# cestpasphoto/alpha-zero-general

Hardware: AMD Instinct MI355X
Metric: self-play env-steps/sec @ numMCTSSims=800, Splendor-2p (higher is better)
Workload: dtype f64

## Files before the change

alpha-zero-general_amd/_lib.py:

```python
import ctypes as C
import os

HERE = os.path.dirname(os.path.abspath(__file__))
LIB_PATH = os.environ.get('AZG_LIB') or os.path.join(HERE, 'libazg_hip.so')

SPLENDOR, SANTORINI, AZUL, MINIVILLES, ABALONE, TLP, BOTANIK, AKROPOLIS, SMALLWORLD = 0, 1, 2, 3, 4, 5, 6, 7, 8


class ForestCfg(C.Structure):
    _fields_ = [('game', C.c_int), ('variant', C.c_int), ('n_trees', C.c_int), ('node_capacity', C.c_int),
                ('row_capacity_bytes', C.c_int), ('numMCTSSims', C.c_int), ('cpuct', C.c_double), ('fpu', C.c_double),
                ('universes', C.c_int), ('prob_fullMCTS', C.c_double), ('ratio_fullMCTS', C.c_int),
                ('forced_playouts', C.c_int), ('dirichletAlpha', C.c_double), ('temperature', C.c_double * 3),
                ('tempThreshold', C.c_double), ('rng_seed', C.c_uint64), ('stream0', C.c_uint64),
                ('max_examples', C.c_int), ('level_budget', C.c_int), ('work_budget', C.c_int), ('gc_high_water_pct', C.c_int)]


class SelfplayStats(C.Structure):
    _fields_ = [(n, C.c_uint64) for n in ('plies', 'games', 'sims', 'levels', 'expansions', 'sum_valid_visited',
                                          'terminal_hits', 'examples', 'gc_runs', 'max_nodes', 'errors',
                                          'sum_depth_at_expand', 'cyc_select', 'cyc_levels', 'cyc_edge', 'cyc_leaf')] + [
                                          ('cyc_seg', C.c_uint64 * 4), ('max_live_after_gc', C.c_uint64), ('examples_dropped', C.c_uint64)]


class AzgError(RuntimeError):
    pass


_lib = None

EXPORTS = [
    'azg_last_error', 'azg_version', 'azg_device_count', 'azg_set_device', 'azg_game_info', 'azg_env_valid_moves',
    'azg_env_next_state', 'azg_env_game_ended', 'azg_env_canonical', 'azg_env_init_boards', 'azg_env_symmetries', 'azg_env_symmetries_ex', 'azg_debug_poison_onchip', 'azg_stream_create_xcd', 'azg_stream_destroy', 'azg_debug_placement', 'azg_eval_hashnet', 'azg_forest_create',
    'azg_forest_destroy', 'azg_forest_device_bytes', 'azg_forest_reset', 'azg_forest_begin_search',
    'azg_forest_select', 'azg_forest_select_fused', 'azg_forest_rounds_v80_h2', 'azg_forest_rounds_profile', 'azg_forest_expand_backup', 'azg_forest_active', 'azg_forest_action_probs',
    'azg_forest_root_stats', 'azg_forest_dump_tree', 'azg_forest_validate', 'azg_selfplay_start', 'azg_selfplay_start_ex', 'azg_selfplay_advance', 'azg_selfplay_active',
    'azg_selfplay_stats_get', 'azg_selfplay_drain_examples', 'azg_forest_last_kernel_ms', 'azg_forest_enable_timing', 'azg_forest_set_search_params', 'azg_nn_v80_forward', 'azg_nn_v80_forward_split', 'azg_nn_v80_forward_h2',
    'azg_nn_mb1d_forward', 'azg_nn_mb1d_forward_h2', 'azg_nn_conv5_forward', 'azg_nn_conv5_forward_split', 'azg_nn_conv5_forward_h2', 'azg_nn_s78_forward', 'azg_nn_s78_forward_split', 'azg_nn_s78_forward_h2',
    'azg_nn_aba21_forward', 'azg_nn_sw62_forward', 'azg_nn_akr31_forward', 'azg_nn_bot_forward', 'azg_forest_async_rounds_sw62', 'azg_pick_actions', 'azg_env_playouts',
    'azg_eval_losses', 'azg_train_sample_ids', 'azg_train_gather', 'azg_train_losses',
    'azg_train_adamw', 'azg_train_step_advance', 'azg_examples_expand', 'azg_train_gather_forms',
]


def lib():
    global _lib
    if _lib is not None:
        return _lib
    if not os.path.exists(LIB_PATH):
        raise AzgError('HIP extension %s is missing: run `python __graft_entry__.py build` (hipcc, gfx950). '
                       'There is no CPU fallback.' % LIB_PATH)
    L = C.CDLL(LIB_PATH)
    vp, i, u64, dbl = C.c_void_p, C.c_int, C.c_uint64, C.c_double
    ip = C.POINTER(C.c_int)
    L.azg_last_error.restype = C.c_char_p
    L.azg_version.restype = C.c_char_p
    if hasattr(L, 'azg_forest_cfg_size') and L.azg_forest_cfg_size() != C.sizeof(ForestCfg):
        raise AzgError('%s (%s) has a %d-byte azg_forest_cfg, this binding a %d-byte one: rebuild the library'
                       % (LIB_PATH, L.azg_version().decode(), L.azg_forest_cfg_size(), C.sizeof(ForestCfg)))
    L.azg_game_info.argtypes = [i, i, ip, ip, ip, ip, ip]
    L.azg_env_valid_moves.argtypes = [i, i, vp, vp, i, vp, vp]
    L.azg_env_next_state.argtypes = [i, i, vp, vp, vp, vp, i, vp, vp, u64, u64, vp, vp]
    L.azg_env_game_ended.argtypes = [i, i, vp, vp, i, vp, vp, vp, vp]
    L.azg_env_canonical.argtypes = [i, i, vp, vp, i, vp, vp]
# ... 97 lines not shown
```

alpha-zero-general_amd/csrc/azg_async.hip.h:

```cpp
#pragma once
#include "azg_fused.hip.h"
#include "selfplay.hip.h"

namespace azg {

constexpr uint32_t ERR_ASYNC_TIMEOUT = 128;
constexpr int ASYNC_RING_LAPS = 8;
#ifndef AZG_ASYNC_SEL_WAVES
#define AZG_ASYNC_SEL_WAVES 16
#endif
constexpr int ASYNC_SEL_WAVES = AZG_ASYNC_SEL_WAVES;
#ifndef AZG_ASYNC_SCOUTS
#define AZG_ASYNC_SCOUTS 1
#endif
constexpr uint32_t ASYNC_IDLE_STEP_CAP = 100000u;
#ifndef AZG_IDLE_SLEEP
#define AZG_IDLE_SLEEP 16
#endif
#ifndef AZG_SCOUT_SLEEP
#define AZG_SCOUT_SLEEP 8
#endif
#ifndef AZG_V80_NET_SHARE_256
#define AZG_V80_NET_SHARE_256 136
#endif
// ... 644 lines not shown
                astore(A->ts_ready + (size_t)gi * ASYNC_RS + ii, wall32());
                astore(A->ready + (size_t)gi * ASYNC_RS + ii, (uint32_t)sidx[16 + tid] + 1u);
            }
        }
        if (tid == 0) {
            P[0] += 1ull; P[1] += (unsigned long long)sidx[32]; P[2] += (unsigned long long)(wall32() - (uint32_t)sidx[33]);
            P[5] += (unsigned long long)((uint32_t)clock64() - (uint32_t)sidx[37]);
        }
    }
    if (threadIdx.x == 0) {
        const AsyncArgsC A = (AsyncArgsC)(uintptr_t)args;
        unsigned long long* prof = A->prof;
        atomicAdd(prof + 3, P[0]); atomicAdd(prof + 4, P[1]); atomicAdd(prof + 5, P[2]); atomicAdd(prof + 6, P[3]);
        atomicAdd(prof + 7, P[4]); atomicAdd(prof + 11, (unsigned long long)(wall32() - t_begin)); atomicAdd(prof + 14, P[5]);
        unsigned long long* wi = A->wginfo + (size_t)(A->n_sel + (int)blockIdx.x) * 4;
        wi[0] = where_am_i(); wi[1] = 2ull | ((unsigned long long)(wall32() - t_begin) << 8); wi[2] += P[0]; wi[3] += P[5];
        if (blockIdx.x == 0) { const uint32_t ab = aload(&A->ctl->abort); if (ab == 1u || ab == 2u) atomicAdd(prof + 16 + ab, 1ull); else if (ab == 0u) prof[19] = 0ull; }
        unsigned long long* dn = A->wginfo + (size_t)4 * 1024 + 280 + 2 * (size_t)blockIdx.x;
        dn[0] = (unsigned long long)(uint32_t)sidx[34] | ((unsigned long long)(uint32_t)sidx[35] << 32);
        dn[1] = (unsigned long long)(uint32_t)sidx[36] | ((unsigned long long)(uint32_t)sidx[32] << 32);
    }
}

#endif
}

#ifndef AZG_MV_NET_SHARE_256
#define AZG_MV_NET_SHARE_256 128
#endif
#ifndef AZG_TLP_NET_SHARE_256
#define AZG_TLP_NET_SHARE_256 160
#endif
#ifdef AZG_ASYNC_SANTORINI11
#define AZG_ASYNC_KIND_SANTORINI11(X) X(SantoriniDev<11>, NetNone, AZG_SANTORINI, 11, "Santorini with gods", "Santorini with gods only", WT_C5, 196, false, ASYNC_NO_GEOMETRY)
#else
#define AZG_ASYNC_KIND_SANTORINI11(X)
#endif
#define AZG_ASYNC_KINDS(X) \
    X(SplendorDev<2>, NetV80, AZG_SPLENDOR, 2, "Splendor 2 players", "Splendor 2 players only (the V80 geometry of nn_v80_h2.hip.h)", WT_V80, AZG_V80_NET_SHARE_256, false, ASYNC_NO_GEOMETRY)  \
    X(SantoriniDev<1>, NetC5, AZG_SANTORINI, 1, "Santorini without gods", "Santorini without gods only (the V89 geometry of nn_conv5x5.hip.h)", WT_C5, 196, false, ASYNC_NO_GEOMETRY)           \
    X(SplendorDev<3>, NetSpl3, AZG_SPLENDOR, 3, "Splendor 3 players", nullptr, WT_MB, 208, false, AZG_NET_SPLENDOR3)                                                                            \
    X(SplendorDev<4>, NetSpl4, AZG_SPLENDOR, 4, "Splendor 4 players", nullptr, WT_MB, 208, false, AZG_NET_SPLENDOR4)                                                                            \
    X(AzulDev, NetAzul, AZG_AZUL, -1, "Azul", nullptr, WT_MB, 104, false, AZG_NET_AZUL)                                                                                                         \
    X(SmallworldDev<2>, NetSw62<2>, AZG_SMALLWORLD, 2, "Smallworld 2 players", "Smallworld only (the V62 geometry of nn_smallworld.hip.h)", WT_SW, 224, true, ASYNC_NO_GEOMETRY)                \
    X(SmallworldDev<3>, NetSw62<3>, AZG_SMALLWORLD, 3, "Smallworld 3 players", "Smallworld only (the V62 geometry of nn_smallworld.hip.h)", WT_SW, 224, true, ASYNC_NO_GEOMETRY)                \
    X(SmallworldDev<4>, NetSw62<4>, AZG_SMALLWORLD, 4, "Smallworld 4 players", "Smallworld only (the V62 geometry of nn_smallworld.hip.h)", WT_SW, 224, true, ASYNC_NO_GEOMETRY)                \
// ... 25 lines not shown
int azg_async_launch_select(int net_kind, const azg::AsyncArgs* devbuf, int n_sel, hipStream_t s);
struct AsyncSlot {
    AsyncArgs host; AsyncArgs* devbuf;
    int8_t* aleaf; AsyncCtl* ctl; unsigned long long* ring; uint32_t* ready; uint32_t* ts; uint32_t* evald; uint8_t* pending; uint32_t* carry; unsigned long long* prof; unsigned long long* wginfo;
    hipEvent_t fork, join, join_net;
    int n_sel, n_net, ring_bits;
    int device, n_cu, leaf_stride, T;
};
constexpr const char* ASYNC_SLOT_KEY = "async_pipeline";
static void async_slot_free(void* p) {
    AsyncSlot* s = (AsyncSlot*)p;
    (void)hipFree(s->devbuf); (void)hipFree(s->aleaf); (void)hipFree(s->ctl); (void)hipFree(s->ring); (void)hipFree(s->ready);
    (void)hipFree(s->ts); (void)hipFree(s->evald); (void)hipFree(s->pending); (void)hipFree(s->carry); (void)hipFree(s->prof); (void)hipFree(s->wginfo);
    if (s->fork) (void)hipEventDestroy(s->fork);
    if (s->join) (void)hipEventDestroy(s->join);
    if (s->join_net) (void)hipEventDestroy(s->join_net);
    delete s;
}

struct AsyncDevice { int n_cu; hipStream_t net_stream, sel_stream; bool attr_done; };
constexpr int ASYNC_MAX_DEVICES = 64;
static AsyncDevice g_async_dev[ASYNC_MAX_DEVICES];

extern "C" int azg_forest_async_profile(azg_forest* f, double* out , int reset) {
    if (!f || !out) return fail("azg_forest_async_profile: null argument");
    for (int i = 0; i < ASYNC_NPROF; i++) out[i] = 0.0;
    AsyncSlot* sl = (AsyncSlot*)azg_forest_attached(f, ASYNC_SLOT_KEY);
    if (!sl) return 0;
    HIPCHK(hipDeviceSynchronize());
    unsigned long long h[ASYNC_NPROF];
    HIPCHK(hipMemcpy(h, sl->prof, sizeof(h), hipMemcpyDeviceToHost));
    for (int i = 0; i < ASYNC_NPROF; i++) out[i] = (double)h[i];
    out[12] = (double)sl->n_sel; out[13] = (double)sl->n_net;
    {
        AsyncCtl c;
        HIPCHK(hipMemcpy(&c, sl->ctl, sizeof(c), hipMemcpyDeviceToHost));
        out[20] = (double)c.leaf_tail; out[21] = (double)c.leaf_head; out[22] = (double)c.retired; out[23] = (double)c.abort;
        out[24] = (double)c.calls; out[25] = (double)c.stop;
    }
    if (reset) HIPCHK(hipMemset(sl->prof, 0, sizeof(h)));
    return 0;
}

extern "C" int azg_forest_async_wginfo(azg_forest* f, unsigned long long* out , int max_wg, int reset) {
    if (!f || !out) return fail("azg_forest_async_wginfo: null argument");
    AsyncSlot* sl = (AsyncSlot*)azg_forest_attached(f, ASYNC_SLOT_KEY);
// ... 16 lines not shown
    if (ring_out) HIPCHK(hipMemcpy(ring_out, sl->ring, sizeof(unsigned long long) * (size_t)(max_ring < (1 << sl->ring_bits) ? max_ring : (1 << sl->ring_bits)), hipMemcpyDeviceToHost));
    return sl->ring_bits;
}

__global__ __launch_bounds__(256) void k_async_requeue(const AsyncArgs* args) {
    const AsyncArgsC A = (AsyncArgsC)(uintptr_t)args;
    const int t = (int)(blockIdx.x * blockDim.x + threadIdx.x);
    if (t >= A->F.T) return;
    const bool owed = aload(A->evald + t) == 0u && aload(&A->F.hdr[t].status) == ST_WAIT_NN && !aload(&A->F.hdr[t].err);
    A->pending[t] = owed ? (uint8_t)1 : (uint8_t)0;
    if (owed) {
        const uint32_t rb = (uint32_t)A->ring_bits, tk = atomicAdd(&A->ctl->leaf_tail, 1u);
        const uint32_t calls = (uint32_t)A->rounds + (A->total_calls ? 0u : A->carry[t]);
        if (!A->total_calls) A->carry[t] = calls;
        A->ring[tk & ((1u << rb) - 1u)] = (unsigned long long)((uint32_t)t | (((wall32() >> 4) & 0xFFFu) << 20)) | ((unsigned long long)calls << 32) |
                                           ((unsigned long long)(((tk >> rb) & 7u) + 1u) << 60);
        atomicAdd(A->prof + 27, 1ull);
    }
}

template <class NET>
static int async_launch_net(const AsyncArgs* devbuf, int n_net, hipStream_t s) {
    return launch_lds<k_async_net<NET>>(dim3(n_net), dim3(768), NET::LDS + ASYNC_DESC_BYTES, s, devbuf);
}
enum AsyncWt { WT_V80, WT_C5, WT_MB, WT_SW };
constexpr int ASYNC_NO_GEOMETRY = -1;
using AsyncNetLaunch = int (*)(const AsyncArgs*, int, hipStream_t);
struct AsyncKind {
    int game, variant; const char* name; const char* only; int leaf_stride, bs, wt, net_256; bool cap_trees; int geometry; const char* geometry_name;
    AsyncNetLaunch launch_net, launch_hashnet;
};
static_assert(AsyncLeaf<SplendorDev<2>>::STRIDE == H2_AL_STRIDE && AsyncLeaf<SplendorDev<2>>::MASK_OFF == H2_AL_MASK, "leaf record layout shared with the net kernel");
static_assert(AsyncLeaf<SantoriniDev<1>>::STRIDE == C5_AL_STRIDE && AsyncLeaf<SantoriniDev<1>>::MASK_OFF == C5_AL_MASK, "leaf record layout shared with the net kernel");
#ifdef AZG_ASYNC_SANTORINI11
struct NetNone { static constexpr int BS = 16; };
template <> int async_launch_net<NetNone>(const AsyncArgs*, int, hipStream_t) { return fail("no engine net for this game in the pipeline"); }
#endif
#define X(G, NET, GAME, VARIANT, NAME, ONLY, WT, NET_256, CAP_TREES, GEOMETRY)                                                                  \
    {GAME, VARIANT, NAME, ONLY, AsyncLeaf<G>::STRIDE, NET::BS, WT, NET_256, CAP_TREES, GEOMETRY, #GEOMETRY, &async_launch_net<NET>, &async_launch_net<NetHash<G>>},
static const AsyncKind ASYNC_KINDS[] = {AZG_ASYNC_KINDS(X)};
#undef X
constexpr int ASYNC_NKINDS = (int)(sizeof(ASYNC_KINDS) / sizeof(ASYNC_KINDS[0]));
static int async_kind_of_game(int game, int variant) {
    for (int k = 0; k < ASYNC_NKINDS; k++)
        if (ASYNC_KINDS[k].game == game && (ASYNC_KINDS[k].variant < 0 || ASYNC_KINDS[k].variant == variant)) return k;
    return -1;
// ... 219 lines not shown
```

alpha-zero-general_amd/csrc/nn_v80_h2.hip.h:

```cpp
#pragma once
#include "nn_kernels.hip.h"

#pragma clang fp contract(on)

namespace azg {

typedef _Float16 f16x8 __attribute__((ext_vector_type(8)));
typedef _Float16 f16x2_t __attribute__((ext_vector_type(2)));

constexpr float H2_AS = 64.f, H2_IAS = 1.f / 64.f;

struct H2BlockW {
    const uint4 *We, *W1, *W2, *Wp;
    const float *be, *Wd, *sd, *bd, *b1, *b2, *bp;
    float se, s1, s2, sp;
};
struct H2NetW {
    const uint4 *W0, *Wpi1, *Wpi2, *Wv1;
    const float *b0, *bpi1, *bpi2, *bv1, *Wv2, *bv2;
    float s0, spi1, spi2, sv1;
};

struct H2Weights { H2BlockW Wt, Wp, Wv; H2NetW N; };
static inline H2Weights h2_weights(const void* const* w, const float* descale) {
// ... 113 lines not shown
__device__ __forceinline__ void h2_load_ew(H2EW& e, const H2BlockW& W, int nt, int g, int lane) {
#pragma unroll
    for (int c = 0; c < 2; c++) { e.weh[c] = H2FRAG(W.We, 2, nt, c, 0); e.wel[c] = H2FRAG(W.We, 2, nt, c, 1); }
    const int ch0 = nt * 16 + 4 * g;
    e.be4 = *H2G(f32x4, W.be + ch0); e.sd4 = *H2G(f32x4, W.sd + ch0); e.bd4 = *H2G(f32x4, W.bd + ch0);
    e.wdv = H2G(float, W.Wd)[lane < 49 ? lane : 0];
}

constexpr int H2_RSX = 128, H2_RSH = 384;
constexpr int H2_XH = 0, H2_XL = 14336, H2_OH = 28672, H2_OL = 43008, H2_HH = 57344, H2_HL = 100352, H2_PLH = 143360, H2_PLL = 149504,
              H2_SHH = 155648, H2_SHL = 157696, H2_LDS = 159744;
constexpr int H2_PDX = H2_XL - H2_XH, H2_PDH = H2_HL - H2_HH, H2_PDP = H2_PLL - H2_PLH, H2_PDS = H2_SHL - H2_SHH;
constexpr int H2_RED = H2_HH, H2_HIDH = H2_HH + 12288, H2_HIDL = H2_HIDH + 6144, H2_LG = H2_HIDL + 6144, H2_LS = 100;

#ifdef AZG_NN_PHASE_TIMES
static __device__ long long g_h2_phase[4][16];
#define H2_PH(k) do { if (blockIdx.x == 7 && threadIdx.x == 0) g_h2_phase[MODE][k] = clock64(); } while (0)
#else
#define H2_PH(k)
#endif

constexpr int H2_AL_STRIDE = 416, H2_AL_MASK = 400;
constexpr int H2_IND_MASK = 52;
template <int ACT, int POOLMAX, int MODE, int NW, bool IND = false>
__device__ __forceinline__ void h2_block(uint8_t* lds, const H2BlockW& W, const H2NetW& N, int B, int P,
                                         const uint8_t* __restrict__ valid, float* __restrict__ pi_out, float* __restrict__ v_out,
                                         H2EW& ew ,
                                         const H2BlockW& Wnext, int wg, const int tid, const int* sidx = nullptr) {
    constexpr int NS = 16, A = 81;
    constexpr bool LEAN = NW > 12;
    const int lane = tid & 63, wave = tid >> 6;
    const int g = lane >> 4, r = lane & 15;
    const int b0 = wg * NS;
    uint8_t* const XH = lds + H2_XH;
    uint8_t* const OH = lds + H2_OH;
    uint8_t* const HH = lds + H2_HH;
    uint8_t* const PLH = lds + H2_PLH;
    uint8_t* const SHH = lds + H2_SHH;
    H2_PH(0);

    const int nt = wave < 11 ? wave : 0;
    uint4 w2h[2], w2l[2];
    const int ch0 = nt * 16 + 4 * g;
    const uint4 weh0 = ew.weh[0], weh1 = ew.weh[1], wel0 = ew.wel[0], wel1 = ew.wel[1];
    const f32x4 be4 = ew.be4, sd4 = ew.sd4, bd4 = ew.bd4;
    const float wdv = ew.wdv;
    const int cs1 = tid / 12, cc1 = 4 * (tid - cs1 * 12);
    f32x4 b24, b14;
    if (tid < 448) {
        const int row = tid >> 2, q = 22 + (tid & 1), pl = (tid >> 1) & 1;
        *(uint4*)(HH + pl * H2_PDH + h2_off(row, q, H2_RSH)) = make_uint4(0u, 0u, 0u, 0u);
// ... 110 lines not shown
#pragma unroll
        for (int c = 0; c < 2; c++) {
            const int off = h2_off(r, 4 * c + g, H2_RSX);
            acc = h2_mma(w2h[c], w2l[c], *(const uint4*)(SHH + off), *(const uint4*)(SHH + H2_PDS + off), acc);
        }
        const f32x4 y = acc * W.s2 + b24;
        const f32x4 sc = f32x4{hardsigmoid(y[0]), hardsigmoid(y[1]), hardsigmoid(y[2]), hardsigmoid(y[3])};
        const f32x4 scm = sc * (H2_AS / (ACT == ACT_HSWISH ? 6.f : 1.f));
#pragma unroll
        for (int t = 0; t < 7; t++) {
#ifndef AZG_H2_NO_EPRIO
            if (t == 0) __builtin_amdgcn_s_setprio(2);
            if (t == 3) __builtin_amdgcn_s_setprio(1);
            if (t == 6) __builtin_amdgcn_s_setprio(0);
#endif
            h2_store4(HH, H2_PDH, H2_RSH, t * 16 + r, ch0, dw[t] * scm, 1.f);
        }
    };

    if (!LEAN) {
        uint4 w1h[2], w1l[2];
        const int nt1 = wave % 3, kg1 = wave < 9 ? wave / 3 : 0;
        if (wave < 11) phase_e(w1h, w1l, nt1, kg1);
        if (wave < 4 * PG) load_wp();
        else bp4 = *H2G(f32x4, W.bp + ntp * 16 + 4 * g);
        __syncthreads();
        H2_PH(1);
        if (wave < 9) s1_unit(w1h, w1l, nt1, kg1);
        H2_PH(13);
        H2_PH(14);
        __syncthreads();
        H2_PH(15);
        if (tid < 192) s1_combine();
        __syncthreads();
        H2_PH(2);
        if (wave < 11) phase_s2();
        __syncthreads();
        H2_PH(3);
    } else if (wave < 11) {
        uint4 none_h[2], none_l[2];
        if (tid < 192) b14 = *H2G(f32x4, W.b1 + cc1);
        phase_e(none_h, none_l, 0, 0);
        __syncthreads();
        H2_PH(1);
        __syncthreads();
        H2_PH(15);
        if (tid < 192) s1_combine();
        __syncthreads();
        H2_PH(2);
        load_wp();
        phase_s2();
        __syncthreads();
        H2_PH(3);
    } else {
        uint4 w1h[2][2], w1l[2][2];
        const int u0 = wave - 11, u1 = wave - 6;
#pragma unroll
        for (int c = 0; c < 2; c++) { w1h[0][c] = H2FRAG(W.W1, 6, u0 % 3, 2 * (u0 / 3) + c, 0); w1l[0][c] = H2FRAG(W.W1, 6, u0 % 3, 2 * (u0 / 3) + c, 1); }
        if (u1 < 9) {
// ... 136 lines not shown
                    acc = h2_mma(wfh[cc], wfl[cc], *(const uint4*)(OH + off), *(const uint4*)(OH + H2_PDX + off), acc);
                }
            }
            *(f32x4*)(RED + (wave * 16 + r) * 16 + 4 * g) = acc;
        }
        __syncthreads();
        if (tid < NS * P) {
            const int s = tid / P, p = tid - s * P, b = IND ? sidx[s] : b0 + s;
            if (IND ? b >= 0 : b < B) {
                float a = H2G(float, N.bv2)[p];
                for (int j = 0; j < P; j++) {
                    float h = 0.f;
                    for (int w = 0; w < 12; w++) h += RED[(w * 16 + s) * 16 + j];
                    a += fmaxf(h * N.sv1 + H2G(float, N.bv1)[j], 0.f) * H2G(float, N.Wv2)[j * P + p];
                }
                if constexpr (IND) __hip_atomic_store((uint32_t*)v_out + (size_t)b * P + p, __float_as_uint(tanhf(a)), __ATOMIC_RELAXED, __HIP_MEMORY_SCOPE_AGENT);
                else v_out[(size_t)b * P + p] = tanhf(a);
            }
        }
        H2_PH(5);
    }
}

template <int NW, bool IND = false>
__device__ __forceinline__ void h2_net_body(uint8_t* lds, H2WeightsC Wc, const int8_t* __restrict__ boards, const uint8_t* __restrict__ valid,
                                            int B, int P, float* __restrict__ pi_out, float* __restrict__ v_out, int wg, const int* sidx = nullptr) {
    constexpr int NS = 16, C = 56, NT = NW * 64, KB = (NS * (7 * C / 4) + NT - 1) / NT;
    h2_fp16_saturate_mode();
    int tid_ = threadIdx.x;
    asm volatile("" : "+v"(tid_));
    const int tid = tid_, lane = tid & 63, wave = tid >> 6;
    const int g = lane >> 4, r = lane & 15;
    const int b0 = wg * NS;
    const int nb = min(NS, B - b0);
    uint8_t* const XH = lds + H2_XH;
    uint8_t* const X0 = lds + H2_OH;

    const uint32_t* bsrc = (const uint32_t*)(boards + (size_t)b0 * (7 * C));
    uint32_t bv[KB];
    unsigned long long ind_mask = 0ull;
    if constexpr (IND) {
        if (tid < 32) {
            const int b = sidx[tid >> 1];
            if (b >= 0) ind_mask = __hip_atomic_load((const unsigned long long*)(valid + (size_t)b * H2_AL_STRIDE + H2_AL_MASK) + (tid & 1), __ATOMIC_RELAXED,
                                                     __HIP_MEMORY_SCOPE_AGENT);
        }
    }
#pragma unroll
    for (int k = 0; k < KB; k++) {
        const int i = tid + NT * k;
        if constexpr (IND) {
            const int s = i / (7 * C / 4), d = i - s * (7 * C / 4);
            const int b = i < NS * (7 * C / 4) ? sidx[s] : -1;
            bv[k] = b >= 0 ? __hip_atomic_load((const uint32_t*)(boards + (size_t)b * H2_AL_STRIDE) + d, __ATOMIC_RELAXED, __HIP_MEMORY_SCOPE_AGENT) : 0u;
        } else
            bv[k] = (i < NS * (7 * C / 4) && i / (7 * C / 4) < nb) ? bsrc[i] : 0u;
    }
    constexpr int RG0 = NW / 4;
    const int ntp = wave & 3, rt0 = wave >> 2;
    uint4 w0h[2], w0l[2];
    float s0;
    f32x4 b04;
    H2EW ew;
    {
        const H2WeightsC c0 = h2_opaque(Wc);
        const H2NetW N = h2_load_const(&c0->N);
        const H2BlockW Wt = h2_load_const(&c0->Wt);
#pragma unroll
        for (int c = 0; c < 2; c++) { w0h[c] = H2FRAG(N.W0, 2, ntp, c, 0); w0l[c] = H2FRAG(N.W0, 2, ntp, c, 1); }
        b04 = *H2G(f32x4, N.b0 + ntp * 16 + 4 * g);
        s0 = N.s0;
        h2_load_ew(ew, Wt, wave < 11 ? wave : 0, g, lane);
    }
    if (tid < 768) *(uint4*)(lds + H2_PLH + tid * 16) = make_uint4(0u, 0u, 0u, 0u);
    if (tid < 256) *(uint4*)(lds + H2_SHH + tid * 16) = make_uint4(0u, 0u, 0u, 0u);
    if (tid < 112) *(uint4*)(X0 + h2_off(tid, 7, H2_RSX)) = make_uint4(0u, 0u, 0u, 0u);
    if constexpr (IND) { if (tid < 32) ((unsigned long long*)(sidx + H2_IND_MASK))[tid] = ind_mask; }
    __syncthreads();
#pragma unroll
    for (int k = 0; k < KB; k++) {
        const int i = tid + NT * k;
        if (i < NS * (7 * C / 4)) {
            const int s = i / (7 * C / 4), d = i - s * (7 * C / 4);
#pragma unroll
            for (int q = 0; q < 4; q++) {
                const int idx = 4 * d + q, c = idx / 7, l = idx - c * 7;
                const _Float16 hv = (_Float16)(float)((int)(int8_t)(bv[k] >> (8 * q)) * 64);
                *(_Float16*)(X0 + h2_off(l * 16 + s, c >> 3, H2_RSX) + ((c & 7) << 1)) = hv;
            }
        }
    }
    __syncthreads();
#pragma unroll 1
    for (int rt = rt0; rt < 7; rt += RG0) {
        const int row = rt * 16 + r;
        f32x4 acc = f32x4{0.f, 0.f, 0.f, 0.f};
#pragma unroll
        for (int c = 0; c < 2; c++) {
            const f16x8 a = __builtin_bit_cast(f16x8, *(const uint4*)(X0 + h2_off(row, 4 * c + g, H2_RSX)));
            acc = __builtin_amdgcn_mfma_f32_16x16x32_f16(__builtin_bit_cast(f16x8, w0l[c]), a, acc, 0, 0, 0);
            acc = __builtin_amdgcn_mfma_f32_16x16x32_f16(__builtin_bit_cast(f16x8, w0h[c]), a, acc, 0, 0, 0);
        }
        h2_store4(XH, H2_PDX, H2_RSX, row, ntp * 16 + 4 * g, acc * s0 + b04);
    }
    __syncthreads();
    {
        const H2WeightsC c1 = h2_opaque(Wc);
        const H2BlockW Wt = h2_load_const(&c1->Wt), Wp = h2_load_const(&c1->Wp);
        const H2NetW N = h2_load_const(&c1->N);
        h2_block<1, 0, 1, NW, IND>(lds, Wt, N, B, P, valid, pi_out, v_out, ew, Wp, wg, tid, sidx);
    }
    {
        const H2WeightsC c2 = h2_opaque(Wc);
        const H2BlockW Wp = h2_load_const(&c2->Wp), Wv = h2_load_const(&c2->Wv);
        const H2NetW N = h2_load_const(&c2->N);
        h2_block<2, 1, 2, NW, IND>(lds, Wp, N, B, P, valid, pi_out, v_out, ew, Wv, wg, tid, sidx);
    }
    {
        const H2WeightsC c3 = h2_opaque(Wc);
        const H2BlockW Wv = h2_load_const(&c3->Wv);
        const H2NetW N = h2_load_const(&c3->N);
        h2_block<2, 1, 3, NW, IND>(lds, Wv, N, B, P, valid, pi_out, v_out, ew, Wv, wg, tid, sidx);
    }
}

template <int NW>
__global__ __launch_bounds__(NW * 64) void k_v80_net_h2(H2Weights W ,
                                                        const int8_t* __restrict__ boards, const uint8_t* __restrict__ valid, int B, int P,
                                                        float* __restrict__ pi_out, float* __restrict__ v_out) {
    extern __shared__ __attribute__((aligned(16))) uint8_t lds[];
    const H2WeightsC Wc = (H2WeightsC)__builtin_amdgcn_kernarg_segment_ptr();
    h2_net_body<NW>(lds, Wc, boards, valid, B, P, pi_out, v_out, (int)blockIdx.x);
}

}

#pragma clang fp contract(off)
```

alpha-zero-general_amd/forest.py:

```python
import collections
import ctypes as C

import numpy as np
import torch

from . import _lib
from ._lib import ForestCfg, SelfplayStats, check, lib


def _ptr(t):
    return None if t is None else C.c_void_p(t.data_ptr())


def _stream():
    return C.c_void_p(torch.cuda.current_stream().cuda_stream)


PipelineNet = collections.namedtuple('PipelineNet', 'name match entry head weights')


def _by_class(cls, *flags):
    return lambda n: type(n).__name__ == cls and all(getattr(n, f, False) for f in flags)


# ... 145 lines not shown
                                        int(bool(shared_budget)), _stream()))

    async_rounds_v80 = async_rounds

    def async_counters(self, reset=False):
        out = (C.c_double * 96)()
        check(lib().azg_forest_async_profile(self.h, out, int(reset)))
        return list(out)

    def async_profile(self, reset=True, since=None):
        o = self.async_counters(reset)
        if since is not None:
            o = [a - b if k not in (12, 13) and not 20 <= k < 32 else a for k, (a, b) in enumerate(zip(o, since))]
        d = dict(descents=o[0], batches=o[3], leaves=o[4], launches=o[9], plies_in_kernel=o[16])
        d['descent_us'] = o[1] / max(o[0], 1) / 100.0
        d['forward_us'] = o[5] / max(o[3], 1) / 100.0
        d['leaves_per_batch'] = o[4] / max(o[3], 1)
        d['leaf_wait_us'] = o[7] / max(o[4], 1) / 100.0
        d['ready_wait_us'] = o[8] / max(o[0], 1) / 100.0
        d['select_wave_busy'] = o[1] / max(o[1] + o[2], 1)
        d['net_wg_busy'] = o[5] / max(o[11], 1)
        d['n_sel'], d['n_net'] = int(o[12]), int(o[13])
        d['timeouts'] = dict(select=int(o[17]), net=int(o[18]), ranges_abandoned=int(o[26]), leaves_requeued=int(o[27]))
        d['ctl'] = dict(leaf_tail=int(o[20]), leaf_head=int(o[21]), retired=int(o[22]), abort=int(o[23]), calls=int(o[24]), stop=int(o[25]))
        d['forward_cycles'] = o[14] / max(o[3], 1)
        d['descent_cycles'] = o[15] / max(o[0], 1)
        d['net_cu_mhz'] = o[14] / max(o[5], 1) * 100.0
        d['select_cu_mhz'] = o[15] / max(o[1], 1) * 100.0
        d['launch_us'] = o[10] / max(o[9], 1) / max(o[12], 1) / 100.0
        d['select_resident_ticks'], d['net_resident_ticks'] = o[10], o[11]
        d['leaf_wait_hist_us'] = [int(x) for x in o[32:64]]
        d['ready_wait_hist_us'] = [int(x) for x in o[64:96]]
        return d

    def async_wginfo(self, reset=True):
        buf = (C.c_uint64 * (4 * 1024))()
        n = check(lib().azg_forest_async_wginfo(self.h, buf, 1024, int(reset)))
        out = []
        for k in range(n):
            w, role, calls, cyc = buf[4 * k], buf[4 * k + 1], buf[4 * k + 2], buf[4 * k + 3]
            out.append((int(w & 0xF), int((w >> 8) & 0xF), int((w >> 16) & 0x7), int((w >> 24) & 1), int(role & 0xFF), int(calls), cyc / max(calls, 1),
                        int(role >> 8) / 100.0))
        return out

    def rounds_profile(self, reset=True):
        out = (C.c_double * 4)()
# ... 99 lines not shown
```

include/azg.h:

```cpp
#ifndef AZG_H
#define AZG_H
#include <stdint.h>
#include <stddef.h>

#ifdef __cplusplus
extern "C" {
#endif

enum { AZG_SPLENDOR = 0, AZG_SANTORINI = 1, AZG_AZUL = 2, AZG_MINIVILLES = 3, AZG_ABALONE = 4, AZG_TLP = 5, AZG_BOTANIK = 6, AZG_AKROPOLIS = 7, AZG_SMALLWORLD = 8 };
#define AZG_MAX_PLAYERS 5
#define AZG_MAX_UNIVERSES 8

const char* azg_last_error(void);
const char* azg_version(void);
int azg_device_count(void);
int azg_set_device(int device);

int azg_game_info(int game, int variant, int* state_bytes, int* action_size, int* num_players, int* rows, int* cols);

int azg_env_valid_moves(int game, int variant, const int8_t* states_dev, const int32_t* players_dev, int n,
                        uint8_t* out_valid_dev, void* stream);
int azg_env_next_state(int game, int variant, const int8_t* states_dev, const int32_t* players_dev,
                       const int32_t* actions_dev, const int64_t* random_seeds_dev, int n, int8_t* out_states_dev,
                       int32_t* out_next_players_dev, uint64_t rng_seed, uint64_t stream0, uint64_t* counters_dev,
// ... 95 lines not shown

int azg_forest_begin_search(azg_forest* f, const int8_t* roots_dev, const uint8_t* full_dev, void* stream);
int azg_forest_select(azg_forest* f, int8_t* leaf_states_dev, uint8_t* leaf_valid_dev, uint8_t* needs_eval_dev,
                      const double* root_noise_dev , int noise_stride, void* stream);
int azg_forest_select_fused(azg_forest* f, int8_t* leaf_states_dev, uint8_t* leaf_valid_dev, uint8_t* needs_eval_dev,
                            const float* pi_dev, const float* v_dev, int noise_stride, void* stream);
int azg_forest_rounds_v80_h2(azg_forest* f, int8_t* leaf_states_dev, uint8_t* leaf_valid_dev, uint8_t* needs_eval_dev, float* pi_dev,
                             float* v_dev, int noise_stride, const void* const* w, const float* descale_host, int rounds, void* stream);
int azg_forest_rounds_profile(azg_forest* f, double* out4, int reset);

int azg_forest_async_rounds_v80_h2(azg_forest* f, uint8_t* leaf_valid_dev, uint8_t* needs_eval_dev, float* pi_dev, float* v_dev,
                                   int noise_stride, const void* const* w, const float* descale_host, int rounds, int n_net, int n_sel,
                                   int batch_wait_ticks, int shared_budget, void* stream);
int azg_forest_async_rounds_conv5_h2(azg_forest* f, uint8_t* leaf_valid_dev, uint8_t* needs_eval_dev, float* pi_dev, float* v_dev,
                                     int noise_stride, const float* const* w, float descale, int rounds, int n_net, int n_sel,
                                     int batch_wait_ticks, int shared_budget, void* stream);
int azg_forest_async_rounds_mb1d_h2(azg_forest* f, int geometry, uint8_t* leaf_valid_dev, uint8_t* needs_eval_dev, float* pi_dev, float* v_dev,
                                    int noise_stride, const void* const* w, const float* descale_host, int rounds, int n_net, int n_sel,
                                    int batch_wait_ticks, int shared_budget, void* stream);
int azg_forest_async_rounds_sw62(azg_forest* f, uint8_t* leaf_valid_dev, uint8_t* needs_eval_dev, float* pi_dev, float* v_dev, int noise_stride,
                                 const float* const* w, int rounds, int n_net, int n_sel, int batch_wait_ticks, int shared_budget, void* stream);
#define AZG_ASYNC_NPROF 96
int azg_forest_async_profile(azg_forest* f, double* out96, int reset);

int azg_forest_expand_backup(azg_forest* f, const float* pi_dev, const float* v_dev, const double* root_noise_dev,
                             int noise_stride, void* stream);
int azg_forest_active(azg_forest* f, int* n_active);
int azg_forest_action_probs(azg_forest* f, double temp, double* probs_dev, float* q_dev, uint8_t* is_full_dev,
                            void* stream);
int azg_forest_root_stats(azg_forest* f, int32_t* Ns_dev, float* Qs_dev, int32_t* Nsa_dev, double* Qsa_dev,
                          float* Ps_dev, int32_t* n_nodes_dev, void* stream);
int azg_forest_dump_tree(azg_forest* f, int tree, int max_nodes, int8_t* states, int32_t* Ns, float* Qs, float* Es,
                         int32_t* Nsa, double* Qsa, float* Ps, uint8_t* has_policy);

int azg_stream_create_xcd(int xcd_first, int xcd_count, void** out_stream);
int azg_stream_destroy(void* stream);
int azg_forest_validate(azg_forest* f, int verbose);

int azg_selfplay_start(azg_forest* f, const int8_t* init_boards_dev , void* stream);
int azg_selfplay_start_ex(azg_forest* f, const int8_t* init_boards_dev , uint64_t epoch, int64_t episode_quota,
                          void* stream);
int azg_forest_cfg_size(void);
int azg_selfplay_advance(azg_forest* f, void* stream);
int azg_selfplay_active(azg_forest* f, int* n_active);
typedef struct azg_selfplay_stats {
    uint64_t plies, games, sims, levels, expansions, sum_valid_visited, terminal_hits, examples, gc_runs, max_nodes,
// ... 57 lines not shown
```

Baseline: 44810.

## Prestage next V80 batch during current forward pass in async net kernel

Adds a specialized async net kernel for Splendor-2p (V80) that double-buffers batch descriptors. While the current batch's forward pass runs, a spare wave claims the next ring range, polls briefly for a full batch, and loads its leaf boards and masks into LDS under the phase_e/phase_s2 hooks. A full next batch then skips the separate staging pass and the ring-poll latency. The kernel also hoists weight requests across iterations, at the cost of more LDS, extra hook logic in the network block, and short polling stalls on wave 11.

```diff
diff --git a/alpha-zero-general_amd/_lib.py b/alpha-zero-general_amd/_lib.py
--- a/alpha-zero-general_amd/_lib.py
+++ b/alpha-zero-general_amd/_lib.py
@@ -40,6 +40,7 @@
     'azg_nn_aba21_forward', 'azg_nn_sw62_forward', 'azg_nn_akr31_forward', 'azg_nn_bot_forward', 'azg_forest_async_rounds_sw62', 'azg_pick_actions', 'azg_env_playouts',
     'azg_eval_losses', 'azg_train_sample_ids', 'azg_train_gather', 'azg_train_losses',
     'azg_train_adamw', 'azg_train_step_advance', 'azg_examples_expand', 'azg_train_gather_forms',
+    'azg_async_v80_net_lds_bytes',
 ]
 
 
diff --git a/alpha-zero-general_amd/csrc/azg_async.hip.h b/alpha-zero-general_amd/csrc/azg_async.hip.h
--- a/alpha-zero-general_amd/csrc/azg_async.hip.h
+++ b/alpha-zero-general_amd/csrc/azg_async.hip.h
@@ -690,6 +690,244 @@
     }
 }
 
+constexpr int V80_DESC_BYTES = 2 * ASYNC_DESC_BYTES, V80_STAMPS = H2_IND_MASK + 16 * 2 * 2;
+static_assert((V80_STAMPS + 16) * 4 <= ASYNC_DESC_BYTES, "the stamps fit the descriptor");
+constexpr int V80_NET_LDS_BYTES = NetV80::LDS + V80_DESC_BYTES;
+static_assert(V80_NET_LDS_BYTES <= 160 * 1024, "V80 net LDS + two batch descriptors");
+static_assert(16 * H2_BOARD_DWORDS * 4 <= H2_SHH - H2_PLH && 16 * H2_BOARD_DWORDS % 4 == 0, "the fetched records fit the PL planes, in whole 16-byte units");
+struct V80Prestage {
+    static constexpr bool ON = true;
+    static constexpr int BS = NetV80::BS, NREC = (BS * H2_BOARD_DWORDS + 63) / 64;
+    static constexpr uint32_t FULL = (1u << BS) - 1u;
+    static constexpr uint32_t POLL_TICKS = 120u;
+    const AsyncArgs* args;
+    uint8_t* lds;
+    int* cw;
+    int* nxt;
+    int tid;
+    template <int MODE>
+    __device__ __forceinline__ void under_phase_e(const int wave) {
+        if constexpr (MODE == 2) {
+            if (wave == 11 && (tid & 63) == 0 && !cw[36]) {
+                const uint32_t b = atomicAdd(&((AsyncArgsC)(uintptr_t)args)->ctl->leaf_head, (uint32_t)BS);
+                cw[34] = (int)b; cw[35] = 0; cw[36] = 1;
+            }
+        }
+        if constexpr (MODE == 3) {
+            drain_vmem();
+            if (wave != 11) return;
+            const AsyncArgsC A = (AsyncArgsC)(uintptr_t)args;
+            const int lane = tid & 63;
+            const uint32_t t0 = wall32();
+            const uint32_t rb = (uint32_t)A->ring_bits, rmask = (1u << rb) - 1u;
+            const uint32_t tk = (uint32_t)cw[34] + (uint32_t)(lane % BS), tag = ((tk >> rb) & 7u) + 1u;
+            unsigned long long e = 0ull;
+            bool pre = false;
+            if (cw[36] && cw[35] == 0) {
+                for (;;) {
+                    e = lane < BS ? __hip_atomic_load(A->ring + (tk & rmask), __ATOMIC_RELAXED, __HIP_MEMORY_SCOPE_AGENT) : 0ull;
+                    if (((uint32_t)__ballot(lane < BS && (uint32_t)(e >> 60) == tag)) == FULL) { pre = true; break; }
+                    if (wall32() - t0 >= POLL_TICKS) break;
+                    __builtin_amdgcn_s_sleep(1);
+                }
+            }
+            if (pre && lane < BS) {
+                nxt[lane] = (int)((uint32_t)e & 0xFFFFFu);
+                nxt[16 + lane] = (int)((e >> 32) & 0xFFFFFFu);
+                nxt[V80_STAMPS + lane] = (int)(uint32_t)e;
+            }
+            if (lane == 0) cw[38] = pre ? 1 : 0;
+        }
+    }
+    template <int MODE>
+    __device__ __forceinline__ void under_phase_s2(const int wave) {
+        if constexpr (MODE == 3) {
+            if (wave != 11 || !cw[38]) return;
+            const uint8_t* const leaf = (const uint8_t*)((AsyncArgsC)(uintptr_t)args)->aleaf;
+            const int lane = tid & 63;
+            uint32_t rec[NREC];
+            unsigned long long msk = 0ull;
+            if (lane < 32) msk = __hip_atomic_load((const unsigned long long*)(leaf + (size_t)nxt[lane >> 1] * H2_AL_STRIDE + H2_AL_MASK) + (lane & 1), __ATOMIC_RELAXED,
+                                                   __HIP_MEMORY_SCOPE_AGENT);
+#pragma unroll
+            for (int k = 0; k < NREC; k++) {
+                const int i = lane + 64 * k, s = i / H2_BOARD_DWORDS, d = i - s * H2_BOARD_DWORDS;
+                rec[k] = s < BS ? __hip_atomic_load((const uint32_t*)(leaf + (size_t)nxt[s] * H2_AL_STRIDE) + d, __ATOMIC_RELAXED, __HIP_MEMORY_SCOPE_AGENT) : 0u;
+            }
+            uint32_t* const raw = (uint32_t*)(lds + H2_PLH);
+#pragma unroll
+            for (int k = 0; k < NREC; k++)
+                if (lane + 64 * k < BS * H2_BOARD_DWORDS) raw[lane + 64 * k] = rec[k];
+            if (lane < 32) ((unsigned long long*)(nxt + H2_IND_MASK))[lane] = msk;
+        }
+    }
+};
+
+template <>
+__global__ __launch_bounds__(768) void k_async_net<NetV80>(const AsyncArgs* args) {
+    extern __shared__ __attribute__((aligned(256))) uint8_t lds[];
+    using NET = NetV80;
+    constexpr int BS = NET::BS;
+    constexpr uint32_t FULL = (1u << BS) - 1u;
+    int* const sidx = (int*)(lds + NET::LDS);
+    const uint32_t t_begin = wall32();
+    unsigned long long* const P = (unsigned long long*)(lds + NET::LDS + 160);
+    if ((int)threadIdx.x < 6) P[threadIdx.x] = 0ull;
+    if (threadIdx.x == 0) { sidx[36] = 0; sidx[38] = 0; sidx[39] = 0; }
+    H2First first;
+    h2_net_parts<12, true, H2_REQUEST>(lds, &((AsyncArgsC)(uintptr_t)args)->W, nullptr, nullptr, 0, 0, nullptr, nullptr, 0, nullptr, first, (int)threadIdx.x);
+    int par = 0;
+    int tid_ = (int)threadIdx.x;
+    __syncthreads();
+#pragma unroll 1
+    for (;;) {
+        asm volatile("" : "+v"(tid_));
+        const int tid = tid_, wave = __builtin_amdgcn_readfirstlane(tid >> 6), lane = tid & 63;
+        int* const cur = sidx + par * (ASYNC_DESC_BYTES / 4);
+        const bool pre = sidx[38] != 0;
+        if (wave == 0 && pre) {
+            if (lane == 0) { sidx[32] = BS; sidx[35] = (int)FULL; sidx[36] = 0; sidx[39] += 1; }
+        } else if (wave == 0) {
+            const AsyncArgsC A = (AsyncArgsC)(uintptr_t)args;
+            AsyncCtl* const ctl = A->ctl;
+            const int T = A->F.T, wait_ticks = A->batch_wait, timeout = A->timeout_ticks;
+            const uint32_t rb = (uint32_t)A->ring_bits, rmask = (1u << rb) - 1u;
+            const uint32_t idle0 = wall32();
+            uint32_t idle_acc = 0u, idle_last = idle0;
+            uint32_t base = (uint32_t)sidx[34], taken = (uint32_t)sidx[35];
+            if (!sidx[36]) {
+                uint32_t b = 0u;
+                if (lane == 0) b = atomicAdd(&ctl->leaf_head, (uint32_t)BS);
+                base = uni_u32(b); taken = 0u;
+            }
+            uint32_t tk = base + (uint32_t)(lane % BS);
+            uint32_t tag = ((tk >> rb) & 7u) + 1u;
+            uint32_t first_seen = 0u;
+            unsigned long long e = 0ull;
+            bool seen = false;
+            int n = 0;
+            uint32_t take = 0u;
+            unsigned spins = 0u;
+            for (;;) {
+                e = lane < BS ? __hip_atomic_load(A->ring + (tk & rmask), __ATOMIC_RELAXED, __HIP_MEMORY_SCOPE_AGENT) : 0ull;
+                const uint32_t filled = (uint32_t)__ballot(lane < BS && (uint32_t)(e >> 60) == tag) & ~taken;
+                if ((uint32_t)__ballot(lane < BS && (uint32_t)(e >> 60) == ((((tk >> rb) + 1u) & 7u) + 1u)) & ~taken) {
+                    uint32_t b = 0u;
+                    if (lane == 0) { b = atomicAdd(&ctl->leaf_head, (uint32_t)BS); atomicAdd(A->prof + 26, 1ull); }
+                    base = uni_u32(b); taken = 0u;
+                    tk = base + (uint32_t)(lane % BS); tag = ((tk >> rb) & 7u) + 1u;
+                    seen = false;
+                    continue;
+                }
+                const uint32_t now = wall32();
+                { const uint32_t d = now - idle_last; idle_acc += d < ASYNC_IDLE_STEP_CAP ? d : ASYNC_IDLE_STEP_CAP; idle_last = now; }
+                if (filled && !seen) { seen = true; first_seen = now; }
+                if (filled && ((filled | taken) == FULL || (int)(now - first_seen) >= wait_ticks)) { take = filled; n = __popc(filled); break; }
+                if (!filled && (++spins & 7u) == 0u) {
+                    if (uni_u32(aload(&ctl->retired)) >= (uint32_t)T || uni_u32(aload(&ctl->abort))) { n = -1; break; }
+                    if (idle_acc > (uint32_t)timeout) {
+                        if (lane == 0) {
+                            astore(&ctl->abort, 2u);
+                            if (atomicAdd(A->prof + 19, 1ull) >= 7ull) atomicOr(&A->F.hdr[0].err, ERR_ASYNC_TIMEOUT);
+                        }
+                        n = -1;
+                        break;
+                    }
+                }
+                if (filled) __builtin_amdgcn_s_sleep(1); else __builtin_amdgcn_s_sleep(4);
+            }
+            if (n > 0) {
+                const uint32_t now = wall32();
+                taken |= take;
+                if (lane < 16) { cur[lane] = -1; cur[16 + lane] = 0; }
+                const bool mine = lane < BS && ((take >> lane) & 1u);
+                uint32_t w = 0u;
+                if (mine) {
+                    const int slot = __popc(take & ((1u << lane) - 1u));
+                    cur[slot] = (int)((uint32_t)e & 0xFFFFFu);
+                    cur[16 + slot] = (int)((e >> 32) & 0xFFFFFFu);
+                    w = ((((now >> 4) & 0xFFFu) - (((uint32_t)e >> 20) & 0xFFFu)) & 0xFFFu) << 4;
+                    atomicAdd(A->prof + 32 + ((w / 100u) < 31u ? (w / 100u) : 31u), 1ull);
+                }
+#pragma unroll
+                for (int m = 8; m >= 1; m >>= 1) w += __shfl_xor(w, m, 16);
+                if (lane == 0) {
+                    P[4] += (unsigned long long)w; P[3] += (unsigned long long)(now - idle0);
+                    sidx[34] = (int)base; sidx[35] = (int)taken; sidx[36] = taken != FULL ? 1 : 0;
+                }
+            }
+            if (lane == 0) sidx[32] = n;
+        }
+        __syncthreads();
+        if (sidx[32] < 0) break;
+        if (tid == 0) { sidx[33] = (int)wall32(); sidx[37] = (int)(uint32_t)clock64(); }
+        par ^= 1;
+        {
+            const AsyncArgs* a = args;
+            asm volatile("" : "+s"(a));
+            const AsyncArgsC A = (AsyncArgsC)(uintptr_t)a;
+            V80Prestage hk;
+            hk.args = a; hk.lds = lds; hk.cw = sidx; hk.nxt = sidx + par * (ASYNC_DESC_BYTES / 4); hk.tid = tid;
+            h2_fp16_saturate_mode();
+            if (!pre) h2_net_parts<12, true, H2_STAGE>(lds, &A->W, A->aleaf, (const uint8_t*)A->aleaf, A->F.T, NET::G::P, A->pi, A->v, 0, cur, first, tid);
+            h2_net_parts<12, true, H2_FORWARD, V80Prestage>(lds, &A->W, A->aleaf, (const uint8_t*)A->aleaf, A->F.T, NET::G::P, A->pi, A->v, 0, cur, first, tid, &hk);
+        }
+            h2_net_parts<12, true, H2_REQUEST>(lds, &((AsyncArgsC)(uintptr_t)args)->W, nullptr, nullptr, 0, 0, nullptr, nullptr, 0, nullptr, first, tid);
+        if (wave == 0) {
+            const AsyncArgsC A = (AsyncArgsC)(uintptr_t)args;
+            drain_vmem();
+            if (tid < 16 && cur[tid] >= 0) {
+                const int t = cur[tid], ns = A->n_sel;
+                const int gi = t % ns, ii = t / ns;
+                astore(A->evald + t, 1u);
+                astore(A->ts_ready + (size_t)gi * ASYNC_RS + ii, wall32());
+                astore(A->ready + (size_t)gi * ASYNC_RS + ii, (uint32_t)cur[16 + tid] + 1u);
+            }
+            if (tid == 0) {
+                P[0] += 1ull; P[1] += (unsigned long long)sidx[32]; P[2] += (unsigned long long)(wall32() - (uint32_t)sidx[33]);
+                P[5] += (unsigned long long)((uint32_t)clock64() - (uint32_t)sidx[37]);
+            }
+        } else if (sidx[38]) {
+#pragma unroll
+            for (int k = 0; k < 2; k++) {
+                const int u = tid - 64 + 704 * k;
+                if (u < BS * H2_BOARD_DWORDS / 4) {
+                    const uint4 v = ((const uint4*)(lds + H2_PLH))[u];
+                    const uint32_t w4[4] = {v.x, v.y, v.z, v.w};
+#pragma unroll
+                    for (int q = 0; q < 4; q++) { const int i = 4 * u + q, s = i / H2_BOARD_DWORDS; h2_scatter_board(lds + H2_OH, s, i - s * H2_BOARD_DWORDS, w4[q]); }
+                }
+                h2_zero_pad(lds, u);
+            }
+            if (wave == 11) {
+                const AsyncArgsC A = (AsyncArgsC)(uintptr_t)args;
+                const uint32_t now = wall32();
+                uint32_t w = 0u;
+                if (lane < BS) {
+                    w = ((((now >> 4) & 0xFFFu) - (((uint32_t)(sidx + par * (ASYNC_DESC_BYTES / 4))[V80_STAMPS + lane] >> 20) & 0xFFFu)) & 0xFFFu) << 4;
+                    atomicAdd(A->prof + 32 + ((w / 100u) < 31u ? (w / 100u) : 31u), 1ull);
+                }
+#pragma unroll
+                for (int m = 8; m >= 1; m >>= 1) w += __shfl_xor(w, m, 16);
+                if (lane == 0) P[4] += (unsigned long long)w;
+            }
+        }
+    }
+    if (threadIdx.x == 0) {
+        const AsyncArgsC A = (AsyncArgsC)(uintptr_t)args;
+        unsigned long long* prof = A->prof;
+        atomicAdd(prof + 3, P[0]); atomicAdd(prof + 4, P[1]); atomicAdd(prof + 5, P[2]); atomicAdd(prof + 6, P[3]);
+        atomicAdd(prof + 7, P[4]); atomicAdd(prof + 11, (unsigned long long)(wall32() - t_begin)); atomicAdd(prof + 14, P[5]);
+        atomicAdd(prof + 28, (unsigned long long)sidx[39]);
+        unsigned long long* wi = A->wginfo + (size_t)(A->n_sel + (int)blockIdx.x) * 4;
+        wi[0] = where_am_i(); wi[1] = 2ull | ((unsigned long long)(wall32() - t_begin) << 8); wi[2] += P[0]; wi[3] += P[5];
+        if (blockIdx.x == 0) { const uint32_t ab = aload(&A->ctl->abort); if (ab == 1u || ab == 2u) atomicAdd(prof + 16 + ab, 1ull); else if (ab == 0u) prof[19] = 0ull; }
+        unsigned long long* dn = A->wginfo + (size_t)4 * 1024 + 280 + 2 * (size_t)blockIdx.x;
+        dn[0] = (unsigned long long)(uint32_t)sidx[34] | ((unsigned long long)(uint32_t)sidx[35] << 32);
+        dn[1] = (unsigned long long)(uint32_t)sidx[36] | ((unsigned long long)(uint32_t)sidx[32] << 32);
+    }
+}
+
 #endif
 }
 
@@ -761,6 +999,7 @@
 constexpr int ASYNC_MAX_DEVICES = 64;
 static AsyncDevice g_async_dev[ASYNC_MAX_DEVICES];
 
+extern "C" int azg_async_v80_net_lds_bytes(void) { return V80_NET_LDS_BYTES; }
 extern "C" int azg_forest_async_profile(azg_forest* f, double* out , int reset) {
     if (!f || !out) return fail("azg_forest_async_profile: null argument");
     for (int i = 0; i < ASYNC_NPROF; i++) out[i] = 0.0;
@@ -823,6 +1062,10 @@
 template <class NET>
 static int async_launch_net(const AsyncArgs* devbuf, int n_net, hipStream_t s) {
     return launch_lds<k_async_net<NET>>(dim3(n_net), dim3(768), NET::LDS + ASYNC_DESC_BYTES, s, devbuf);
+}
+template <>
+int async_launch_net<NetV80>(const AsyncArgs* devbuf, int n_net, hipStream_t s) {
+    return launch_lds<k_async_net<NetV80>>(dim3(n_net), dim3(768), V80_NET_LDS_BYTES, s, devbuf);
 }
 enum AsyncWt { WT_V80, WT_C5, WT_MB, WT_SW };
 constexpr int ASYNC_NO_GEOMETRY = -1;
diff --git a/alpha-zero-general_amd/csrc/nn_v80_h2.hip.h b/alpha-zero-general_amd/csrc/nn_v80_h2.hip.h
--- a/alpha-zero-general_amd/csrc/nn_v80_h2.hip.h
+++ b/alpha-zero-general_amd/csrc/nn_v80_h2.hip.h
@@ -159,11 +159,12 @@
 
 constexpr int H2_AL_STRIDE = 416, H2_AL_MASK = 400;
 constexpr int H2_IND_MASK = 52;
-template <int ACT, int POOLMAX, int MODE, int NW, bool IND = false>
+struct H2NoHooks { static constexpr bool ON = false; };
+template <int ACT, int POOLMAX, int MODE, int NW, bool IND = false, class HK = H2NoHooks>
 __device__ __forceinline__ void h2_block(uint8_t* lds, const H2BlockW& W, const H2NetW& N, int B, int P,
                                          const uint8_t* __restrict__ valid, float* __restrict__ pi_out, float* __restrict__ v_out,
                                          H2EW& ew ,
-                                         const H2BlockW& Wnext, int wg, const int tid, const int* sidx = nullptr) {
+                                         const H2BlockW& Wnext, int wg, const int tid, const int* sidx = nullptr, HK* hk = nullptr) {
     constexpr int NS = 16, A = 81;
     constexpr bool LEAN = NW > 12;
     const int lane = tid & 63, wave = tid >> 6;
@@ -320,6 +321,7 @@
         uint4 w1h[2], w1l[2];
         const int nt1 = wave % 3, kg1 = wave < 9 ? wave / 3 : 0;
         if (wave < 11) phase_e(w1h, w1l, nt1, kg1);
+        if constexpr (HK::ON) hk->template under_phase_e<MODE>(wave);
         if (wave < 4 * PG) load_wp();
         else bp4 = *H2G(f32x4, W.bp + ntp * 16 + 4 * g);
         __syncthreads();
@@ -333,6 +335,7 @@
         __syncthreads();
         H2_PH(2);
         if (wave < 11) phase_s2();
+        if constexpr (HK::ON) hk->template under_phase_s2<MODE>(wave);
         __syncthreads();
         H2_PH(3);
     } else if (wave < 11) {
@@ -515,14 +518,34 @@
     }
 }
 
-template <int NW, bool IND = false>
-__device__ __forceinline__ void h2_net_body(uint8_t* lds, H2WeightsC Wc, const int8_t* __restrict__ boards, const uint8_t* __restrict__ valid,
-                                            int B, int P, float* __restrict__ pi_out, float* __restrict__ v_out, int wg, const int* sidx = nullptr) {
+struct H2First {
+    uint4 w0h[2], w0l[2];
+    float s0;
+    f32x4 b04;
+    H2EW ew;
+};
+constexpr int H2_BOARD_DWORDS = 7 * 56 / 4;
+__device__ __forceinline__ void h2_zero_pad(uint8_t* lds, const int i) {
+    uint8_t* const X0 = lds + H2_OH;
+    if (i < 768) *(uint4*)(lds + H2_PLH + i * 16) = make_uint4(0u, 0u, 0u, 0u);
+    else if (i < 1024) *(uint4*)(lds + H2_SHH + (i - 768) * 16) = make_uint4(0u, 0u, 0u, 0u);
+    else if (i < 1136) *(uint4*)(X0 + h2_off(i - 1024, 7, H2_RSX)) = make_uint4(0u, 0u, 0u, 0u);
+}
+__device__ __forceinline__ void h2_scatter_board(uint8_t* X0, const int s, const int d, const uint32_t v) {
+#pragma unroll
+    for (int q = 0; q < 4; q++) {
+        const int idx = 4 * d + q, c = idx / 7, l = idx - c * 7;
+        const _Float16 hv = (_Float16)(float)((int)(int8_t)(v >> (8 * q)) * 64);
+        *(_Float16*)(X0 + h2_off(l * 16 + s, c >> 3, H2_RSX) + ((c & 7) << 1)) = hv;
+    }
+}
+constexpr int H2_STAGE = 1, H2_REQUEST = 2, H2_FORWARD = 4;
+template <int NW, bool IND, int PARTS, class HK = H2NoHooks>
+__device__ __forceinline__ void h2_net_parts(uint8_t* lds, H2WeightsC Wc, const int8_t* __restrict__ boards, const uint8_t* __restrict__ valid,
+                                             int B, int P, float* __restrict__ pi_out, float* __restrict__ v_out, int wg, const int* sidx, H2First& f,
+                                             const int tid, HK* hk = nullptr) {
     constexpr int NS = 16, C = 56, NT = NW * 64, KB = (NS * (7 * C / 4) + NT - 1) / NT;
-    h2_fp16_saturate_mode();
-    int tid_ = threadIdx.x;
-    asm volatile("" : "+v"(tid_));
-    const int tid = tid_, lane = tid & 63, wave = tid >> 6;
+    const int lane = tid & 63, wave = tid >> 6;
     const int g = lane >> 4, r = lane & 15;
     const int b0 = wg * NS;
     const int nb = min(NS, B - b0);
@@ -532,7 +555,7 @@
     const uint32_t* bsrc = (const uint32_t*)(boards + (size_t)b0 * (7 * C));
     uint32_t bv[KB];
     unsigned long long ind_mask = 0ull;
-    if constexpr (IND) {
+    if constexpr (IND && (PARTS & H2_STAGE) != 0) {
         if (tid < 32) {
             const int b = sidx[tid >> 1];
             if (b >= 0) ind_mask = __hip_atomic_load((const unsigned long long*)(valid + (size_t)b * H2_AL_STRIDE + H2_AL_MASK) + (tid & 1), __ATOMIC_RELAXED,
@@ -540,7 +563,7 @@
         }
     }
 #pragma unroll
-    for (int k = 0; k < KB; k++) {
+    for (int k = 0; k < ((PARTS & H2_STAGE) ? KB : 0); k++) {
         const int i = tid + NT * k;
         if constexpr (IND) {
             const int s = i / (7 * C / 4), d = i - s * (7 * C / 4);
@@ -551,11 +574,11 @@
     }
     constexpr int RG0 = NW / 4;
     const int ntp = wave & 3, rt0 = wave >> 2;
-    uint4 w0h[2], w0l[2];
-    float s0;
-    f32x4 b04;
-    H2EW ew;
-    {
+    uint4 (&w0h)[2] = f.w0h, (&w0l)[2] = f.w0l;
+    float& s0 = f.s0;
+    f32x4& b04 = f.b04;
+    H2EW& ew = f.ew;
+    if constexpr ((PARTS & H2_REQUEST) != 0) {
         const H2WeightsC c0 = h2_opaque(Wc);
         const H2NetW N = h2_load_const(&c0->N);
         const H2BlockW Wt = h2_load_const(&c0->Wt);
@@ -565,6 +588,7 @@
         s0 = N.s0;
         h2_load_ew(ew, Wt, wave < 11 ? wave : 0, g, lane);
     }
+    if constexpr ((PARTS & H2_STAGE) != 0) {
     if (tid < 768) *(uint4*)(lds + H2_PLH + tid * 16) = make_uint4(0u, 0u, 0u, 0u);
     if (tid < 256) *(uint4*)(lds + H2_SHH + tid * 16) = make_uint4(0u, 0u, 0u, 0u);
     if (tid < 112) *(uint4*)(X0 + h2_off(tid, 7, H2_RSX)) = make_uint4(0u, 0u, 0u, 0u);
@@ -584,6 +608,8 @@
         }
     }
     __syncthreads();
+    }
+    if constexpr ((PARTS & H2_FORWARD) == 0) return;
 #pragma unroll 1
     for (int rt = rt0; rt < 7; rt += RG0) {
         const int row = rt * 16 + r;
@@ -601,20 +627,29 @@
         const H2WeightsC c1 = h2_opaque(Wc);
         const H2BlockW Wt = h2_load_const(&c1->Wt), Wp = h2_load_const(&c1->Wp);
         const H2NetW N = h2_load_const(&c1->N);
-        h2_block<1, 0, 1, NW, IND>(lds, Wt, N, B, P, valid, pi_out, v_out, ew, Wp, wg, tid, sidx);
+        h2_block<1, 0, 1, NW, IND, HK>(lds, Wt, N, B, P, valid, pi_out, v_out, ew, Wp, wg, tid, sidx, hk);
     }
     {
         const H2WeightsC c2 = h2_opaque(Wc);
         const H2BlockW Wp = h2_load_const(&c2->Wp), Wv = h2_load_const(&c2->Wv);
         const H2NetW N = h2_load_const(&c2->N);
-        h2_block<2, 1, 2, NW, IND>(lds, Wp, N, B, P, valid, pi_out, v_out, ew, Wv, wg, tid, sidx);
+        h2_block<2, 1, 2, NW, IND, HK>(lds, Wp, N, B, P, valid, pi_out, v_out, ew, Wv, wg, tid, sidx, hk);
     }
     {
         const H2WeightsC c3 = h2_opaque(Wc);
         const H2BlockW Wv = h2_load_const(&c3->Wv);
         const H2NetW N = h2_load_const(&c3->N);
-        h2_block<2, 1, 3, NW, IND>(lds, Wv, N, B, P, valid, pi_out, v_out, ew, Wv, wg, tid, sidx);
-    }
+        h2_block<2, 1, 3, NW, IND, HK>(lds, Wv, N, B, P, valid, pi_out, v_out, ew, Wv, wg, tid, sidx, hk);
+    }
+}
+template <int NW, bool IND = false>
+__device__ __forceinline__ void h2_net_body(uint8_t* lds, H2WeightsC Wc, const int8_t* __restrict__ boards, const uint8_t* __restrict__ valid,
+                                            int B, int P, float* __restrict__ pi_out, float* __restrict__ v_out, int wg, const int* sidx = nullptr) {
+    h2_fp16_saturate_mode();
+    int tid_ = threadIdx.x;
+    asm volatile("" : "+v"(tid_));
+    H2First f;
+    h2_net_parts<NW, IND, H2_STAGE | H2_REQUEST | H2_FORWARD>(lds, Wc, boards, valid, B, P, pi_out, v_out, wg, sidx, f, tid_);
 }
 
 template <int NW>
diff --git a/alpha-zero-general_amd/forest.py b/alpha-zero-general_amd/forest.py
--- a/alpha-zero-general_amd/forest.py
+++ b/alpha-zero-general_amd/forest.py
@@ -191,6 +191,7 @@
         d['net_wg_busy'] = o[5] / max(o[11], 1)
         d['n_sel'], d['n_net'] = int(o[12]), int(o[13])
         d['timeouts'] = dict(select=int(o[17]), net=int(o[18]), ranges_abandoned=int(o[26]), leaves_requeued=int(o[27]))
+        d['batches_staged_early'] = int(o[28])
         d['ctl'] = dict(leaf_tail=int(o[20]), leaf_head=int(o[21]), retired=int(o[22]), abort=int(o[23]), calls=int(o[24]), stop=int(o[25]))
         d['forward_cycles'] = o[14] / max(o[3], 1)
         d['descent_cycles'] = o[15] / max(o[0], 1)
diff --git a/include/azg.h b/include/azg.h
--- a/include/azg.h
+++ b/include/azg.h
@@ -141,6 +141,7 @@
                                  const float* const* w, int rounds, int n_net, int n_sel, int batch_wait_ticks, int shared_budget, void* stream);
 #define AZG_ASYNC_NPROF 96
 int azg_forest_async_profile(azg_forest* f, double* out96, int reset);
+int azg_async_v80_net_lds_bytes(void);
 
 int azg_forest_expand_backup(azg_forest* f, const float* pi_dev, const float* v_dev, const double* root_noise_dev,
                              int noise_stride, void* stream);
```

Result: no change. 44730 (-0.2%).
